# rg2/DeepFluoroLabeling-IPCAI2020

Measured on AMD Instinct MI355X. Metric: train images/sec, paper U-Net (depth 6, wf 5, BN, strided-conv down, seg + 14-landmark heads), 1x192x192 (8x-downsampled 184x184 padded), higher is better.
Workload: dtype bf16 (bf16 activations, activation gradients and GEMM weight copies in HBM; bf16 MFMA, fp32 accumulate, BatchNorm statistics, losses, weight gradients and master weights); 1 GPU; BASELINE configs[1]: 8x-downsampled, seg + 14-landmark heat-map dual head, batch 16 per GPU, Dice+NCC loss, SGD nesterov; global_batch=16, image=1x192x192, parallelism=dp1, math=bf16s, optimizer=dfl_amd.SGD(momentum 0.9, nesterov, wd 1e-4)

## Files before the change

### deepfluorolabeling-ipcai2020_amd/csrc/bn_elem.hip

```cpp
#include "chan_unit.h"

namespace dfl {

struct RowGeom {
  int UX;
  int gy;
};

static RowGeom row_geom(int C, int W) {
  const int units = C / W;
  RowGeom g;
  g.UX = 1;
  while (g.UX * 2 <= units && g.UX * 2 <= 256) g.UX *= 2;
  g.gy = (int)ceil_div(units, g.UX);
  return g;
}

static int rowblocks(int64_t M, int C) {
  int64_t nb = ceil_div(M * (int64_t)C, 8192);
  if (nb > 2048) nb = 2048;
  if (nb > M) nb = M;
  if (nb < 1) nb = 1;
  return (int)nb;
}

struct RowLane {
  int ux, uy, RY, c;
  bool cok;
  int64_t r0, r1;
};

template <int W>
__device__ __forceinline__ RowLane row_lane(int UX, int rows_per_block, int64_t M, int C) {
  RowLane t;
  t.RY = 256 / UX;
  t.ux = threadIdx.x % UX;
  t.uy = threadIdx.x / UX;
  t.c = (blockIdx.y * UX + t.ux) * W;
  t.cok = t.c < C;
  t.r0 = (int64_t)blockIdx.x * rows_per_block;
  t.r1 = t.r0 + rows_per_block;
  if (t.r1 > M) t.r1 = M;
  return t;
}

template <int NS, int W>
__device__ __forceinline__ void block_colsum(const float (&s)[NS][W], const RowLane& t, int UX, float* out, int C) {
  __shared__ float red[NS][256][W];
#pragma unroll
  for (int n = 0; n < NS; ++n)
#pragma unroll
    for (int j = 0; j < W; ++j) red[n][threadIdx.x][j] = s[n][j];
  __syncthreads();
  if (t.uy == 0 && t.cok) {
#pragma unroll
    for (int n = 0; n < NS; ++n)
#pragma unroll
      for (int j = 0; j < W; ++j) {
        float sum = 0.f;
        for (int y = 0; y < t.RY; ++y) sum += red[n][y * UX + t.ux][j];
        out[(int64_t)n * C + j] = sum;
      }
  }
}

template <int W, bool BF>
__global__ void __launch_bounds__(256) colstats_kernel(const dfl_colstats_args a, int UX, int rows_per_block) {
  using U = ChanUnit<W, BF>;
  const RowLane t = row_lane<W>(UX, rows_per_block, a.M, a.C);
  float s[2][W];
#pragma unroll
  for (int j = 0; j < W; ++j) s[0][j] = s[1][j] = 0.f;
  if (t.cok) {
    for (int64_t r = t.r0 + t.uy; r < t.r1; r += t.RY) {
      float va[W], vb[W];
      U::load(a.a, r * a.lda + t.c, va);
      if (a.b != nullptr) U::load(a.b, r * a.ldb + t.c, vb);
#pragma unroll
      for (int j = 0; j < W; ++j) {
        s[0][j] += va[j];
        s[1][j] = fmaf(va[j], a.b != nullptr ? vb[j] : va[j], s[1][j]);
      }
    }
  }
  block_colsum<2, W>(s, t, UX, a.partials + (int64_t)blockIdx.x * 2 * a.C + t.c, a.C);
}

__device__ __forceinline__ void sum_partials_f64(const float* __restrict__ partials, int nblocks, int C, int cpb,
                                                 double* out1, double* out2, double (*red)[256]) {
  const int cl = threadIdx.x % cpb, rl = threadIdx.x / cpb, lanes = 256 / cpb;
  const int c = blockIdx.x * cpb + cl;
  double s1 = 0.0, s2 = 0.0;
  if (c < C) {
    int r = rl;
    for (; r + 3 * lanes < nblocks; r += 4 * lanes) {
      float v1[4], v2[4];
#pragma unroll
      for (int u = 0; u < 4; ++u) {
        v1[u] = partials[((int64_t)(r + u * lanes) * 2 + 0) * C + c];
        v2[u] = partials[((int64_t)(r + u * lanes) * 2 + 1) * C + c];
      }
      s1 += ((double)v1[0] + (double)v1[1]) + ((double)v1[2] + (double)v1[3]);
      s2 += ((double)v2[0] + (double)v2[1]) + ((double)v2[2] + (double)v2[3]);
    }
    for (; r < nblocks; r += lanes) {
      s1 += (double)partials[((int64_t)r * 2 + 0) * C + c];
      s2 += (double)partials[((int64_t)r * 2 + 1) * C + c];
    }
  }
  for (int off = 32; off >= cpb; off >>= 1) {
    s1 += __shfl_xor(s1, off, 64);
    s2 += __shfl_xor(s2, off, 64);
  }
  const int wave = threadIdx.x >> 6, lane = threadIdx.x & 63;
  if (lane < cpb) {
    red[0][wave * 8 + lane] = s1;
    red[1][wave * 8 + lane] = s2;
  }
  __syncthreads();
  *out1 = (red[0][cl] + red[0][8 + cl]) + (red[0][16 + cl] + red[0][24 + cl]);
  *out2 = (red[1][cl] + red[1][8 + cl]) + (red[1][16 + cl] + red[1][24 + cl]);
}

static inline int finalize_cpb(int C) { return C >= 512 ? 8 : (C >= 256 ? 4 : (C >= 128 ? 2 : 1)); }

__global__ void __launch_bounds__(256) bn_finalize_kernel(const dfl_bn_finalize_args a, int cpb) {
  __shared__ double red[2][256];
  const int c = blockIdx.x * cpb + (threadIdx.x % cpb);
  double s1, s2;
  sum_partials_f64(a.partials, a.nblocks, a.C, cpb, &s1, &s2, red);
  if (threadIdx.x < cpb && c < a.C) {
    const double cnt = (double)a.count;
    const double mean = s1 / cnt;
    double var = s2 / cnt - mean * mean;
    if (var < 0.0) var = 0.0;
    const double invstd = 1.0 / sqrt(var + (double)a.eps);
    const float scale = (float)((double)a.gamma[c] * invstd);
    a.scale[c] = scale;
    a.shift[c] = (float)((double)a.beta[c] - mean * (double)a.gamma[c] * invstd);
    a.save_mean[c] = (float)mean;
    a.save_invstd[c] = (float)invstd;
    if (a.running_mean != nullptr) {
      const double mom = (double)a.momentum;
      const double unbiased = (cnt > 1.0) ? var * cnt / (cnt - 1.0) : var;
      a.running_mean[c] = (float)((1.0 - mom) * (double)a.running_mean[c] + mom * mean);
      a.running_var[c] = (float)((1.0 - mom) * (double)a.running_var[c] + mom * unbiased);
    }
  }
  if (blockIdx.x == 0 && threadIdx.x == 0 && a.num_batches_tracked != nullptr) *a.num_batches_tracked += 1;
}

__global__ void __launch_bounds__(256) bn_finalize_live_kernel(const dfl_bn_live_job* __restrict__ jobs) {
  const dfl_bn_live_job j = jobs[blockIdx.y];
  const int c = blockIdx.x * 256 + threadIdx.x;
  if (c < j.C) {
    float scale, shift;
    double mean, var;
    bn_live_affine(j.totals, j.gamma, j.beta, (double)j.count, j.eps, j.C, c, &scale, &shift, &mean, &var);
    j.scale[c] = scale;
    j.shift[c] = shift;
    j.save_mean[c] = (float)mean;
    j.save_invstd[c] = (float)(1.0 / sqrt(var + (double)j.eps));
    if (j.running_mean != nullptr) {
      const double mom = (double)j.momentum, cnt = (double)j.count;
      const double unbiased = (cnt > 1.0) ? var * cnt / (cnt - 1.0) : var;
      j.running_mean[c] = (float)((1.0 - mom) * (double)j.running_mean[c] + mom * mean);
      j.running_var[c] = (float)((1.0 - mom) * (double)j.running_var[c] + mom * unbiased);
    }
  }
  if (blockIdx.x == 0 && threadIdx.x == 0 && j.num_batches_tracked != nullptr) *j.num_batches_tracked += 1;
}

__global__ void __launch_bounds__(256) bn_bwd_finalize_live_kernel(const dfl_bn_bwd_live_job* __restrict__ jobs) {
  const dfl_bn_bwd_live_job j = jobs[blockIdx.y];
  const int c = blockIdx.x * 256 + threadIdx.x;
  if (c >= j.C) return;
  double sdy = 0.0, sdyr = 0.0;
#pragma unroll
  for (int r = 0; r < DFL_BN_R; ++r) {
    sdy += j.totals[(int64_t)(r * 2 + 0) * j.C + c];
    sdyr += j.totals[(int64_t)(r * 2 + 1) * j.C + c];
  }
  const double mean = (double)j.save_mean[c], invstd = (double)j.save_invstd[c];
  j.dgamma[c] = (float)(invstd * (sdyr - mean * sdy));
  j.dbeta[c] = (float)sdy;
  if (j.sum_out != nullptr) j.sum_out[c] = (float)sdy;
}

__global__ void bn_eval_kernel(const float* __restrict__ gamma, const float* __restrict__ beta,
                               const float* __restrict__ rm, const float* __restrict__ rv, float* __restrict__ scale,
                               float* __restrict__ shift, int C, float eps) {
  const int c = blockIdx.x * blockDim.x + threadIdx.x;
  if (c < C) {
    const float invstd = 1.0f / sqrtf(rv[c] + eps);
    const float s = gamma[c] * invstd;
    scale[c] = s;
    shift[c] = beta[c] - rm[c] * s;
  }
}

__global__ void __launch_bounds__(256) bn_bwd_finalize_kernel(const dfl_bn_bwd_finalize_args a, int cpb) {
  __shared__ double red[2][256];
  const int c = blockIdx.x * cpb + (threadIdx.x % cpb);
  double sdy, sdyr;
  sum_partials_f64(a.partials, a.nblocks, a.C, cpb, &sdy, &sdyr, red);
  if (threadIdx.x < cpb && c < a.C) {
    const double cnt = (double)a.count;
    const double mean = (double)a.save_mean[c], invstd = (double)a.save_invstd[c], g = (double)a.gamma[c];
    const double sdyx = invstd * (sdyr - mean * sdy);
    a.dgamma[c] = (float)sdyx;
    a.dbeta[c] = (float)sdy;
    const double s = g * invstd;
    const double c1 = a.count > 0 ? sdy / cnt : 0.0, c2 = a.count > 0 ? sdyx / cnt : 0.0;
    a.coef[0 * a.C + c] = (float)s;
    a.coef[1 * a.C + c] = (float)(-s * c2 * invstd);
    a.coef[2 * a.C + c] = (float)(-s * c1 + s * c2 * invstd * mean);
  }
}

template <int W, bool BF>
__global__ void __launch_bounds__(256) bn_relu_bwd_kernel(const dfl_bn_relu_bwd_args a, int UX, int rows_per_block) {
  using U = ChanUnit<W, BF>;
  const RowLane t = row_lane<W>(UX, rows_per_block, a.M, a.C);
  const int C = a.C, c = t.c, RY = t.RY;
  float cA[W], cB[W], cC[W], s[1][W];
#pragma unroll
  for (int j = 0; j < W; ++j) {
    cA[j] = 1.f; cB[j] = 0.f; cC[j] = 0.f; s[0][j] = 0.f;
    if (a.coef != nullptr && t.cok) {
      cA[j] = a.coef[c + j];
      cB[j] = a.coef[C + c + j];
      cC[j] = a.coef[2 * C + c + j];
    }
  }
  if (t.cok) {
    auto one = [&](const float* dy, const float* rv, int64_t r) {
      float o[W];
#pragma unroll
      for (int j = 0; j < W; ++j) o[j] = rv[j] > 0.f ? fmaf(cA[j], dy[j], fmaf(cB[j], rv[j], cC[j])) : 0.f;
      if (W == 4 && a.split_out) {
        if constexpr (W == 4) {
          uint2 parts[2];
          split_bf16<2>(make_float4(o[0], o[1], o[2], o[3]), parts);
          *reinterpret_cast<uint4*>(a.dpre + r * a.ldo + c) = make_uint4(parts[0].x, parts[0].y, parts[1].x, parts[1].y);
        }
      } else {
        U::store(a.dpre, r * a.ldo + c, o, o);
      }
#pragma unroll
      for (int j = 0; j < W; ++j) s[0][j] += o[j];
    };
    constexpr int R = (W == 4) ? 2 : 4;
    int64_t r = t.r0 + t.uy;
    for (; r + (R - 1) * RY < t.r1; r += R * RY) {
      float dy[R][W], rv[R][W];
#pragma unroll
      for (int u = 0; u < R; ++u) U::load(a.dy, (r + u * RY) * a.lddy + c, dy[u]);
#pragma unroll
      for (int u = 0; u < R; ++u) U::load(a.r, (r + u * RY) * a.ldr + c, rv[u]);
#pragma unroll
      for (int u = 0; u < R; ++u) one(dy[u], rv[u], r + u * RY);
    }
    for (; r < t.r1; r += RY) {
      float dy[W], rv[W];
      U::load(a.dy, r * a.lddy + c, dy);
      U::load(a.r, r * a.ldr + c, rv);
      one(dy, rv, r);
    }
  }
  if (a.partials == nullptr) return;
  block_colsum<1, W>(s, t, UX, a.partials + (int64_t)blockIdx.x * C + c, C);
}

__global__ void __launch_bounds__(256) reduce_partials_kernel(const float* __restrict__ partials, float* __restrict__ out,
                                                             int nblocks, int stride, int C) {
  __shared__ double red[256];
  const int cl = threadIdx.x & 7, rl = threadIdx.x >> 3;
  const int c = blockIdx.x * 8 + cl;
  double s = 0.0;
  if (c < C)
    for (int r = rl; r < nblocks; r += 32) s += (double)partials[(int64_t)r * stride + c];
  red[threadIdx.x] = s;
  __syncthreads();
  for (int off = 16; off >= 1; off >>= 1) {
    if (rl < off) red[threadIdx.x] += red[threadIdx.x + off * 8];
    __syncthreads();
  }
  if (threadIdx.x < 8 && c < C) out[c] = (float)red[threadIdx.x];
}

#ifndef DFL_RB_O
#define DFL_RB_O 32
#endif
constexpr int RB_T = 256, RB_O = DFL_RB_O, RB_S = 4 * RB_T / RB_O, RB_WIDE_MIN = 32;
static inline int reduce_job_blocks(int64_t n, int count) {
  return (int)(count >= RB_WIDE_MIN ? ceil_div(n, RB_O) : ceil_div(n, 4 * RB_T));
}

__device__ __forceinline__ void rb_load4(const float* __restrict__ p, int64_t i, int64_t n, bool vec, double* a) {
  if (vec) {
    const float4 v = *reinterpret_cast<const float4*>(p + i);
    a[0] += (double)v.x; a[1] += (double)v.y; a[2] += (double)v.z; a[3] += (double)v.w;
  } else {
#pragma unroll
    for (int e = 0; e < 4; ++e)
      if (i + e < n) a[e] += (double)p[i + e];
  }
}

__device__ __forceinline__ void rb_store4(const dfl_reduce_job& j, int64_t i, const double* v) {
#pragma unroll
  for (int e = 0; e < 4; ++e)
    if (i + e < j.n) {
      const int64_t ii = i + e;
      j.dst[j.T > 1 ? (ii % (j.n / j.T)) * j.T + ii / (j.n / j.T) : ii] = (float)v[e];
    }
}

__global__ void __launch_bounds__(RB_T) reduce_batch_kernel(const dfl_reduce_job* __restrict__ jobs, int njobs) {
  __shared__ double red[RB_S][RB_O + 2];
  int lo = 0, hi = njobs - 1;
  while (lo < hi) {
    const int mid = (lo + hi + 1) >> 1;
    if (jobs[mid].first_block <= (int)blockIdx.x) lo = mid; else hi = mid - 1;
  }
  const dfl_reduce_job j = jobs[lo];
  const int b = (int)blockIdx.x - j.first_block;
  const bool vec = (j.n & 3) == 0 && (j.stride & 3) == 0 && (reinterpret_cast<uintptr_t>(j.src) & 15) == 0;
  if (j.count >= RB_WIDE_MIN) {
    const int o4 = threadIdx.x % (RB_O / 4), sl = threadIdx.x / (RB_O / 4);
    const int64_t i = (int64_t)b * RB_O + 4 * o4;
    double a0[4] = {0, 0, 0, 0}, a1[4] = {0, 0, 0, 0}, a2[4] = {0, 0, 0, 0}, a3[4] = {0, 0, 0, 0};
    if (i < j.n) {
      int k = sl;
      if (vec) {
        for (; k + 7 * RB_S < j.count; k += 8 * RB_S) {
          float4 v[8];
#pragma unroll
          for (int u = 0; u < 8; ++u) v[u] = *reinterpret_cast<const float4*>(j.src + (int64_t)(k + u * RB_S) * j.stride + i);
#pragma unroll
          for (int u = 0; u < 8; u += 4) {
            a0[0] += (double)v[u].x; a0[1] += (double)v[u].y; a0[2] += (double)v[u].z; a0[3] += (double)v[u].w;
            a1[0] += (double)v[u + 1].x; a1[1] += (double)v[u + 1].y; a1[2] += (double)v[u + 1].z; a1[3] += (double)v[u + 1].w;
            a2[0] += (double)v[u + 2].x; a2[1] += (double)v[u + 2].y; a2[2] += (double)v[u + 2].z; a2[3] += (double)v[u + 2].w;
            a3[0] += (double)v[u + 3].x; a3[1] += (double)v[u + 3].y; a3[2] += (double)v[u + 3].z; a3[3] += (double)v[u + 3].w;
          }
        }
      }
      for (; k + 3 * RB_S < j.count; k += 4 * RB_S) {
        rb_load4(j.src + (int64_t)k * j.stride, i, j.n, vec, a0);
        rb_load4(j.src + (int64_t)(k + RB_S) * j.stride, i, j.n, vec, a1);
        rb_load4(j.src + (int64_t)(k + 2 * RB_S) * j.stride, i, j.n, vec, a2);
        rb_load4(j.src + (int64_t)(k + 3 * RB_S) * j.stride, i, j.n, vec, a3);
      }
      for (; k < j.count; k += RB_S) rb_load4(j.src + (int64_t)k * j.stride, i, j.n, vec, a0);
    }
#pragma unroll
    for (int e = 0; e < 4; ++e) red[sl][4 * o4 + e] = (a0[e] + a1[e]) + (a2[e] + a3[e]);
    __syncthreads();
    for (int off = RB_S / 2; off >= 1; off >>= 1) {
      if (sl < off) {
#pragma unroll
        for (int e = 0; e < 4; ++e) red[sl][4 * o4 + e] += red[sl + off][4 * o4 + e];
      }
      __syncthreads();
    }
    if (sl == 0 && i < j.n) rb_store4(j, i, &red[0][4 * o4]);
  } else {
    const int64_t i = ((int64_t)b * RB_T + threadIdx.x) * 4;
    if (i < j.n) {
      double s[4] = {0, 0, 0, 0};
      for (int k = 0; k < j.count; ++k) rb_load4(j.src + (int64_t)k * j.stride, i, j.n, vec, s);
      rb_store4(j, i, s);
    }
  }
}

template <int W, bool BF>
__global__ void __launch_bounds__(256) affine_copy_kernel(const dfl_affine_copy_args a, int64_t total_units, int cq) {
  using U = ChanUnit<W, BF>;
  const int64_t stride = (int64_t)gridDim.x * blockDim.x;
  for (int64_t i = (int64_t)blockIdx.x * blockDim.x + threadIdx.x; i < total_units; i += stride) {
    int u, xw, yh, n;
    unit_coords(i, cq, a.W, a.H, &u, &xw, &yh, &n);
    const int c = u * W;
    const int64_t so = (((int64_t)n * a.xH + a.xoy + yh) * a.xW + a.xox + xw) * a.ldx + c;
    const int64_t dof = (((int64_t)n * a.yH + a.yoy + yh) * a.yW + a.yox + xw) * a.ldy + c;
    float v[W];
    U::load(a.x, so, v);
    if (a.scale != nullptr) {
      float sc[W], sh[W];
      if constexpr (W == 4) {
        ChanUnit<4, false>::load(a.scale, c, sc);
        ChanUnit<4, false>::load(a.shift, c, sh);
      } else {
#pragma unroll
        for (int j = 0; j < W; ++j) { sc[j] = a.scale[c + j]; sh[j] = a.shift[c + j]; }
      }
#pragma unroll
      for (int j = 0; j < W; ++j) v[j] = fmaf(v[j], sc[j], sh[j]);
    }
    if (a.accumulate) {
      float o[W];
      U::load(a.y, dof, o);
#pragma unroll
      for (int j = 0; j < W; ++j) v[j] += o[j];
    }
    U::store(a.y, dof, v);
  }
}

__device__ __forceinline__ int64_t pool_src(const dfl_pool_args& a, int n, int oy, int ox, int ld) {
  return (((int64_t)n * a.H + 2 * oy) * a.W + 2 * ox) * ld;
}

template <int W, bool BF>
__global__ void __launch_bounds__(256) maxpool_fwd_kernel(const dfl_pool_args a, int64_t total_units, int cq) {
  using U = ChanUnit<W, BF>;
  const int Ho = a.H / 2, Wo = a.W / 2;
  const int64_t stride = (int64_t)gridDim.x * blockDim.x;
  for (int64_t i = (int64_t)blockIdx.x * blockDim.x + threadIdx.x; i < total_units; i += stride) {
    int u, ox, oy, n;
    unit_coords(i, cq, Wo, Ho, &u, &ox, &oy, &n);
    const int c = u * W;
    const int64_t s00 = pool_src(a, n, oy, ox, a.ldx) + c, s10 = s00 + (int64_t)a.W * a.ldx;
    float v0[W], v1[W], v2[W], v3[W], m[W];
    U::load(a.x, s00, v0);
    U::load(a.x, s00 + a.ldx, v1);
    U::load(a.x, s10, v2);
    U::load(a.x, s10 + a.ldx, v3);
#pragma unroll
    for (int j = 0; j < W; ++j) m[j] = fmaxf(fmaxf(v0[j], v1[j]), fmaxf(v2[j], v3[j]));
    U::store(a.y, (((int64_t)n * Ho + oy) * Wo + ox) * a.ldy + c, m);
  }
}

__device__ __forceinline__ int first_max4(float v0, float v1, float v2, float v3) {
  int k = 0;
  float m = v0;
  if (v1 > m) { m = v1; k = 1; }
  if (v2 > m) { m = v2; k = 2; }
  if (v3 > m) { k = 3; }
  return k;
}

template <int W, bool BF>
__global__ void __launch_bounds__(256) maxpool_bwd_kernel(const dfl_pool_args a, int64_t total_units, int cq) {
  using U = ChanUnit<W, BF>;
  const int Ho = a.H / 2, Wo = a.W / 2;
  const int64_t stride = (int64_t)gridDim.x * blockDim.x;
  for (int64_t i = (int64_t)blockIdx.x * blockDim.x + threadIdx.x; i < total_units; i += stride) {
    int u, ox, oy, n;
    unit_coords(i, cq, Wo, Ho, &u, &ox, &oy, &n);
    const int c = u * W;
    const int64_t s00 = pool_src(a, n, oy, ox, a.ldx) + c, s10 = s00 + (int64_t)a.W * a.ldx;
    const int64_t d00 = pool_src(a, n, oy, ox, a.lddx) + c, d10 = d00 + (int64_t)a.W * a.lddx;
    float v0[W], v1[W], v2[W], v3[W], g[W];
    U::load(a.x, s00, v0);
    U::load(a.x, s00 + a.ldx, v1);
    U::load(a.x, s10, v2);
    U::load(a.x, s10 + a.ldx, v3);
    U::load(a.y, (((int64_t)n * Ho + oy) * Wo + ox) * a.ldy + c, g);
    if constexpr (BF) {
      float e0[W], e1[W], e2[W], e3[W];
      U::load(a.dx, d00, e0);
      U::load(a.dx, d00 + a.lddx, e1);
      U::load(a.dx, d10, e2);
      U::load(a.dx, d10 + a.lddx, e3);
#pragma unroll
      for (int j = 0; j < W; ++j) {
        const int k = first_max4(v0[j], v1[j], v2[j], v3[j]);
        e0[j] += k == 0 ? g[j] : 0.f;
        e1[j] += k == 1 ? g[j] : 0.f;
        e2[j] += k == 2 ? g[j] : 0.f;
        e3[j] += k == 3 ? g[j] : 0.f;
      }
      U::store(a.dx, d00, e0);
      U::store(a.dx, d00 + a.lddx, e1);
      U::store(a.dx, d10, e2);
      U::store(a.dx, d10 + a.lddx, e3);
    } else {
#pragma unroll
      for (int j = 0; j < W; ++j) {
        const int k = first_max4(v0[j], v1[j], v2[j], v3[j]);
        a.dx[(k < 2 ? d00 : d10) + ((k & 1) ? a.lddx : 0) + j] += g[j];
      }
    }
  }
}

constexpr int PK_T = 32, PK_CMAX = 9;

__device__ __forceinline__ float pack_src(const dfl_pack_job& j, int k, int n) {
  int a, b, c;
  if (j.kind == 1) {
    c = k / j.B; b = k - c * j.B; a = n;
  } else if (j.kind == 2) {
    const int cp = k / j.A;
    a = k - cp * j.A; b = n; c = j.flip ? (j.C - 1 - cp) : cp;
  } else {
    a = k; c = n / j.B; b = n - c * j.B;
  }
  return j.src[((int64_t)a * j.B + b) * j.C + c];
}

__device__ __forceinline__ void pack_put(float* dst, int64_t q, int r, float v, int split) {
  if (!split) {
    dst[q * 4 + r] = v;
  } else {
    const __bf16 h = (__bf16)v;
    const __bf16 l = (__bf16)(v - (float)h);
    unsigned short* d16 = reinterpret_cast<unsigned short*>(dst) + q * 8;
    d16[r] = __builtin_bit_cast(unsigned short, h);
    d16[4 + r] = __builtin_bit_cast(unsigned short, l);
  }
}

__global__ void __launch_bounds__(256) pack_kernel(const dfl_pack_job* __restrict__ jobs) {
  __shared__ float tile[PK_T][PK_T * PK_CMAX + 1];
  const dfl_pack_job j = jobs[blockIdx.y];
  const int A = j.A, B = j.B, Cc = j.C;
  const int K = (j.kind == 1) ? Cc * B : (j.kind == 2 ? Cc * A : A);
  const int N = (j.kind == 1) ? A : (j.kind == 2 ? B : Cc * B);
  if (j.split == 2 && Cc <= PK_CMAX && ((j.kind == 1) ? (B % 16 == 0) : (A % 16 == 0))) {
    const int tb = (B + PK_T - 1) / PK_T, ta = (A + PK_T - 1) / PK_T;
    const int run = PK_T * Cc;
    unsigned short* dst16 = reinterpret_cast<unsigned short*>(j.dst);
    for (int tidx = blockIdx.x; tidx < ta * tb; tidx += gridDim.x) {
      const int a0 = (tidx / tb) * PK_T, b0 = (tidx % tb) * PK_T;
      const int nb = min(PK_T, B - b0), na = min(PK_T, A - a0);
      __syncthreads();
      for (int e = threadIdx.x; e < PK_T * run; e += 256) {
        const int ar = e / run, q = e - ar * run;
        if (ar < na && q < nb * Cc) tile[ar][q] = j.src[((int64_t)(a0 + ar) * B + b0) * Cc + q];
      }
      __syncthreads();
      for (int e = threadIdx.x; e < 64 * Cc; e += 256) {
        const int x = e & 31, blk = (e >> 5) & 1, cp = e >> 6;
        float f[16];
        int64_t cell;
        bool ok;
        if (j.kind == 1) {
          ok = x < na && 16 * blk < nb;
#pragma unroll
          for (int r = 0; r < 16; ++r) f[r] = tile[x][(16 * blk + r) * Cc + cp];
          cell = (int64_t)((cp * B + b0) / 16 + blk) * N + a0 + x;
        } else if (j.kind == 2) {
          const int c = j.flip ? (Cc - 1 - cp) : cp;
          ok = x < nb && 16 * blk < na;
#pragma unroll
          for (int r = 0; r < 16; ++r) f[r] = tile[16 * blk + r][x * Cc + c];
          cell = (int64_t)((cp * A + a0) / 16 + blk) * N + b0 + x;
        } else {
          ok = x < nb && 16 * blk < na;
#pragma unroll
          for (int r = 0; r < 16; ++r) f[r] = tile[16 * blk + r][x * Cc + cp];
          cell = (int64_t)(a0 / 16 + blk) * N + cp * B + b0 + x;
        }
        if (ok) {
          u32x4* d = reinterpret_cast<u32x4*>(dst16 + cell * 16);
          d[0] = pack8(f);
          d[1] = pack8(f + 8);
        }
      }
    }
    return;
  }
  if (j.split == 2) {
    const int Kc = (K + 15) / 16;
    const int64_t cells = (int64_t)Kc * N;
    const int64_t stride = (int64_t)gridDim.x * blockDim.x;
    for (int64_t i = (int64_t)blockIdx.x * blockDim.x + threadIdx.x; i < cells; i += stride) {
      const int n = (int)(i % N), kc = (int)(i / N);
      float f[16];
#pragma unroll
      for (int r = 0; r < 16; ++r) {
        const int k = kc * 16 + r;
        f[r] = k < K ? pack_src(j, k, n) : 0.f;
      }
      u32x4* d = reinterpret_cast<u32x4*>(reinterpret_cast<unsigned short*>(j.dst) + i * 16);
      d[0] = pack8(f);
      d[1] = pack8(f + 8);
    }
    return;
  }
  const bool tiled = Cc <= PK_CMAX && ((j.kind == 1) ? (B % 4 == 0) : (A % 4 == 0));
  if (tiled) {
    const int tb = (B + PK_T - 1) / PK_T, ta = (A + PK_T - 1) / PK_T;
    const int run = PK_T * Cc;
    for (int tidx = blockIdx.x; tidx < ta * tb; tidx += gridDim.x) {
      const int a0 = (tidx / tb) * PK_T, b0 = (tidx % tb) * PK_T;
      const int nb = min(PK_T, B - b0), na = min(PK_T, A - a0);
      __syncthreads();
      for (int e = threadIdx.x; e < PK_T * run; e += 256) {
        const int ar = e / run, q = e - ar * run;
        if (ar < na && q < nb * Cc) tile[ar][q] = j.src[((int64_t)(a0 + ar) * B + b0) * Cc + q];
      }
      __syncthreads();
      for (int e = threadIdx.x; e < PK_T * run; e += 256) {
        const int r = e & 3, x = (e >> 2) & 31, rest = e >> 7;
        if (j.kind == 1) {
          const int c = rest >> 3, bq = rest & 7, bb = 4 * bq + r, ar = x;
          if (ar < na && bb < nb)
            pack_put(j.dst, (int64_t)((c * B + b0) / 4 + bq) * N + a0 + ar, r, tile[ar][bb * Cc + c], j.split);
        } else if (j.kind == 2) {
          const int cp = rest >> 3, aq = rest & 7, ar = 4 * aq + r, bb = x;
          const int c = j.flip ? (Cc - 1 - cp) : cp;
          if (ar < na && bb < nb)
            pack_put(j.dst, (int64_t)((cp * A + a0) / 4 + aq) * N + b0 + bb, r, tile[ar][bb * Cc + c], j.split);
        } else {
          const int c = rest >> 3, aq = rest & 7, ar = 4 * aq + r, bb = x;
          if (ar < na && bb < nb)
            pack_put(j.dst, (int64_t)(a0 / 4 + aq) * N + c * B + b0 + bb, r, tile[ar][bb * Cc + c], j.split);
        }
      }
    }
    return;
  }
  const int Kq = (K + 3) / 4;
  const int64_t total = (int64_t)Kq * N * 4;
  const int64_t stride = (int64_t)gridDim.x * blockDim.x;
  for (int64_t i = (int64_t)blockIdx.x * blockDim.x + threadIdx.x; i < total; i += stride) {
    const int r = (int)(i & 3);
    const int64_t t = i >> 2;
    const int n = (int)(t % N), kq = (int)(t / N);
    const int k = 4 * kq + r;
    pack_put(j.dst, i >> 2, r, (k < K) ? pack_src(j, k, n) : 0.f, j.split);
  }
}

__device__ __forceinline__ void pack_emit_cells(const float (*tile)[PK_T * PK_CMAX + 1], unsigned short* dst16, int kind, int flip,
                                                int A, int B, int Cc, int a0, int b0) {
  const int N = (kind == 1) ? A : (kind == 2 ? B : Cc * B);
  for (int e = threadIdx.x; e < 64 * Cc; e += 256) {
    const int x = e & 31, blk = (e >> 5) & 1, cp = e >> 6;
    float f[16];
    int64_t cell;
    if (kind == 1) {
#pragma unroll
      for (int r = 0; r < 16; ++r) f[r] = tile[x][(16 * blk + r) * Cc + cp];
      cell = (int64_t)((cp * B + b0) / 16 + blk) * N + a0 + x;
    } else if (kind == 2) {
      const int c = flip ? (Cc - 1 - cp) : cp;
#pragma unroll
      for (int r = 0; r < 16; ++r) f[r] = tile[16 * blk + r][x * Cc + c];
      cell = (int64_t)((cp * A + a0) / 16 + blk) * N + b0 + x;
    } else {
#pragma unroll
      for (int r = 0; r < 16; ++r) f[r] = tile[16 * blk + r][x * Cc + cp];
      cell = (int64_t)(a0 / 16 + blk) * N + cp * B + b0 + x;
    }
    u32x4* d = reinterpret_cast<u32x4*>(dst16 + cell * 16);
    d[0] = pack8(f);
    d[1] = pack8(f + 8);
  }
}

__device__ __forceinline__ void pack_emit_quads(const float (*tile)[PK_T * PK_CMAX + 1], float* dst, int kind, int flip, int split,
                                                int A, int B, int Cc, int a0, int b0) {
  const int N = (kind == 1) ? A : (kind == 2 ? B : Cc * B);
  const int run = PK_T * Cc;
  for (int e = threadIdx.x; e < PK_T * run; e += 256) {
    const int r = e & 3, x = (e >> 2) & 31, rest = e >> 7;
    if (kind == 1) {
      const int c = rest >> 3, bq = rest & 7, bb = 4 * bq + r, ar = x;
      pack_put(dst, (int64_t)((c * B + b0) / 4 + bq) * N + a0 + ar, r, tile[ar][bb * Cc + c], split);
    } else if (kind == 2) {
      const int cp = rest >> 3, aq = rest & 7, ar = 4 * aq + r, bb = x;
      const int c = flip ? (Cc - 1 - cp) : cp;
      pack_put(dst, (int64_t)((cp * A + a0) / 4 + aq) * N + b0 + bb, r, tile[ar][bb * Cc + c], split);
    } else {
      const int c = rest >> 3, aq = rest & 7, ar = 4 * aq + r, bb = x;
      pack_put(dst, (int64_t)(a0 / 4 + aq) * N + c * B + b0 + bb, r, tile[ar][bb * Cc + c], split);
    }
  }
// ... 391 lines not shown
```

Before: 4681 images/sec.

## Restructure batched partial-sum reduction with wave shuffles and transposed-output staging

Rewrites reduce_batch_kernel, which sums weight-gradient partials. Job lookup becomes a wave ballot instead of a binary search. The wide path now uses a configurable number of slice lanes per wave with shuffle reductions before a smaller LDS tree, and predicated unrolled rounds of loads. A new narrow path for transposed outputs stages results in shared memory so the stores are coalesced, and the plain narrow path unrolls its loads. The aim is to reduce LDS traffic, barrier count, scattered transposed writes and load latency, at the cost of more complex code with inline asm and scheduling barriers.

```diff
diff --git a/deepfluorolabeling-ipcai2020_amd/csrc/bn_elem.hip b/deepfluorolabeling-ipcai2020_amd/csrc/bn_elem.hip
--- a/deepfluorolabeling-ipcai2020_amd/csrc/bn_elem.hip
+++ b/deepfluorolabeling-ipcai2020_amd/csrc/bn_elem.hip
@@ -289,18 +289,32 @@
   if (threadIdx.x < 8 && c < C) out[c] = (float)red[threadIdx.x];
 }
 
-#ifndef DFL_RB_O
-#define DFL_RB_O 32
+#ifndef DFL_RB_P
+#define DFL_RB_P 8
 #endif
-constexpr int RB_T = 256, RB_O = DFL_RB_O, RB_S = 4 * RB_T / RB_O, RB_WIDE_MIN = 32;
+#ifndef DFL_RB_G
+#define DFL_RB_G 1
+#endif
+constexpr int RB_S = 32, RB_P = DFL_RB_P, RB_L = 64 / RB_P, RB_W = RB_S / RB_P, RB_GO = 4 * RB_L, RB_G = DFL_RB_G;
+constexpr int RB_O = RB_GO * RB_G, RB_T = 64 * RB_W * RB_G, RB_WIDE_MIN = 32;
+static_assert((RB_P == 2 || RB_P == 4 || RB_P == 8) && RB_T <= 1024, "2, 4 or 8 slice lanes per wave");
 static inline int reduce_job_blocks(int64_t n, int count) {
   return (int)(count >= RB_WIDE_MIN ? ceil_div(n, RB_O) : ceil_div(n, 4 * RB_T));
 }
 
+__device__ __forceinline__ void rb_add4(double* a, const float4& v) {
+  a[0] += (double)v.x; a[1] += (double)v.y; a[2] += (double)v.z; a[3] += (double)v.w;
+}
+
+__device__ __forceinline__ float4 rb_ld16(const float* p) {
+  typedef float f4 __attribute__((ext_vector_type(4)));
+  const f4 v = *(const f4 __attribute__((address_space(1))) *)(uintptr_t)p;
+  return make_float4(v.x, v.y, v.z, v.w);
+}
+
 __device__ __forceinline__ void rb_load4(const float* __restrict__ p, int64_t i, int64_t n, bool vec, double* a) {
   if (vec) {
-    const float4 v = *reinterpret_cast<const float4*>(p + i);
-    a[0] += (double)v.x; a[1] += (double)v.y; a[2] += (double)v.z; a[3] += (double)v.w;
+    rb_add4(a, rb_ld16(p + i));
   } else {
 #pragma unroll
     for (int e = 0; e < 4; ++e)
@@ -308,69 +322,171 @@
   }
 }
 
+template <int R>
+__device__ __forceinline__ void rb_round(const float* p, const float* q, int64_t stride, int left, double* a0, double* a1,
+                                         double* a2, double* a3) {
+  if (R == 8) asm volatile("; round of eight"); else asm volatile("; round of four");
+  float4 v[R];
+#pragma unroll
+  for (int u = 0; u < R; ++u) v[u] = rb_ld16(u < left ? q + (int64_t)(u * RB_S) * stride : p);
+  __builtin_amdgcn_sched_barrier(0);
+#pragma unroll
+  for (int u = 0; u < R; ++u)
+    asm volatile("" : "+v"(v[u].x), "+v"(v[u].y), "+v"(v[u].z), "+v"(v[u].w));
+#pragma unroll
+  for (int u = 0; u < R; ++u) {
+    v[u].x = u < left ? v[u].x : 0.f; v[u].y = u < left ? v[u].y : 0.f;
+    v[u].z = u < left ? v[u].z : 0.f; v[u].w = u < left ? v[u].w : 0.f;
+  }
+  if (R == 8 && left >= 8) {
+#pragma unroll
+    for (int u = 0; u < R; u += 4) { rb_add4(a0, v[u]); rb_add4(a1, v[u + 1]); rb_add4(a2, v[u + 2]); rb_add4(a3, v[u + 3]); }
+  } else if (left >= 4) {
+    rb_add4(a0, v[0]); rb_add4(a1, v[1]); rb_add4(a2, v[2]); rb_add4(a3, v[3]);
+#pragma unroll
+    for (int u = 4; u < 7 && u < R; ++u) rb_add4(a0, v[u]);
+  } else {
+#pragma unroll
+    for (int u = 0; u < 3; ++u) rb_add4(a0, v[u]);
+  }
+}
+
+__device__ __forceinline__ void rb_walk(const float* p, int64_t stride, int count, double* s) {
+  int k = 0;
+  for (; k + 3 < count; k += 4) {
+    float4 v[4];
+#pragma unroll
+    for (int u = 0; u < 4; ++u) v[u] = rb_ld16(p + (int64_t)(k + u) * stride);
+#pragma unroll
+    for (int u = 0; u < 4; ++u) rb_add4(s, v[u]);
+  }
+  if (k < count) {
+    float4 v[3];
+#pragma unroll
+    for (int u = 0; u < 3; ++u) {
+      v[u] = rb_ld16(p + (int64_t)(k + u < count ? k + u : k) * stride);
+      if (k + u >= count) v[u] = make_float4(0.f, 0.f, 0.f, 0.f);
+    }
+#pragma unroll
+    for (int u = 0; u < 3; ++u) rb_add4(s, v[u]);
+  }
+}
+
 __device__ __forceinline__ void rb_store4(const dfl_reduce_job& j, int64_t i, const double* v) {
-#pragma unroll
-  for (int e = 0; e < 4; ++e)
-    if (i + e < j.n) {
-      const int64_t ii = i + e;
-      j.dst[j.T > 1 ? (ii % (j.n / j.T)) * j.T + ii / (j.n / j.T) : ii] = (float)v[e];
-    }
-}
-
-__global__ void __launch_bounds__(RB_T) reduce_batch_kernel(const dfl_reduce_job* __restrict__ jobs, int njobs) {
-  __shared__ double red[RB_S][RB_O + 2];
-  int lo = 0, hi = njobs - 1;
-  while (lo < hi) {
-    const int mid = (lo + hi + 1) >> 1;
-    if (jobs[mid].first_block <= (int)blockIdx.x) lo = mid; else hi = mid - 1;
-  }
-  const dfl_reduce_job j = jobs[lo];
+  if (j.T > 1) {
+    const int64_t m = j.n / j.T;
+    int64_t t = i / m, r = i - t * m;
+#pragma unroll
+    for (int e = 0; e < 4; ++e)
+      if (i + e < j.n) {
+        j.dst[r * j.T + t] = (float)v[e];
+        if (++r == m) { r = 0; ++t; }
+      }
+  } else if (i + 3 < j.n && (reinterpret_cast<uintptr_t>(j.dst + i) & 15) == 0) {
+    *reinterpret_cast<float4*>(j.dst + i) = make_float4((float)v[0], (float)v[1], (float)v[2], (float)v[3]);
+  } else {
+#pragma unroll
+    for (int e = 0; e < 4; ++e)
+      if (i + e < j.n) j.dst[i + e] = (float)v[e];
+  }
+}
+
+__global__ void __launch_bounds__(RB_T) __attribute__((amdgpu_waves_per_eu(4, 8))) reduce_batch_kernel(const dfl_reduce_job* __restrict__ jobs, int njobs) {
+  __shared__ double red[RB_G][RB_W][RB_GO];
+  const int lane = threadIdx.x & 63, wv = threadIdx.x >> 6;
+  int below = 0;
+  for (int base = 0; base < njobs; base += 64) {
+    const bool le = base + lane < njobs && jobs[base + lane].first_block <= (int)blockIdx.x;
+    below += __popcll(__ballot(le));
+  }
+  const dfl_reduce_job j = jobs[__builtin_amdgcn_readfirstlane(below - 1)];
   const int b = (int)blockIdx.x - j.first_block;
   const bool vec = (j.n & 3) == 0 && (j.stride & 3) == 0 && (reinterpret_cast<uintptr_t>(j.src) & 15) == 0;
   if (j.count >= RB_WIDE_MIN) {
-    const int o4 = threadIdx.x % (RB_O / 4), sl = threadIdx.x / (RB_O / 4);
-    const int64_t i = (int64_t)b * RB_O + 4 * o4;
+    const int o4 = lane % RB_L, w = __builtin_amdgcn_readfirstlane(wv) % RB_W, og = wv / RB_W, sl = w + RB_W * (lane / RB_L);
+    const int64_t i = (int64_t)b * RB_O + RB_GO * og + 4 * o4;
     double a0[4] = {0, 0, 0, 0}, a1[4] = {0, 0, 0, 0}, a2[4] = {0, 0, 0, 0}, a3[4] = {0, 0, 0, 0};
     if (i < j.n) {
       int k = sl;
       if (vec) {
-        for (; k + 7 * RB_S < j.count; k += 8 * RB_S) {
-          float4 v[8];
-#pragma unroll
-          for (int u = 0; u < 8; ++u) v[u] = *reinterpret_cast<const float4*>(j.src + (int64_t)(k + u * RB_S) * j.stride + i);
-#pragma unroll
-          for (int u = 0; u < 8; u += 4) {
-            a0[0] += (double)v[u].x; a0[1] += (double)v[u].y; a0[2] += (double)v[u].z; a0[3] += (double)v[u].w;
-            a1[0] += (double)v[u + 1].x; a1[1] += (double)v[u + 1].y; a1[2] += (double)v[u + 1].z; a1[3] += (double)v[u + 1].w;
-            a2[0] += (double)v[u + 2].x; a2[1] += (double)v[u + 2].y; a2[2] += (double)v[u + 2].z; a2[3] += (double)v[u + 2].w;
-            a3[0] += (double)v[u + 3].x; a3[1] += (double)v[u + 3].y; a3[2] += (double)v[u + 3].z; a3[3] += (double)v[u + 3].w;
-          }
+        const float* p = j.src + i + (int64_t)sl * j.stride;
+        const int mine = (j.count - 1 - sl) / RB_S + 1, most = (j.count - 1 - w) / RB_S + 1;
+        for (int done = 0; done < most; done += 8) {
+          const float* q = p + (int64_t)(done * RB_S) * j.stride;
+          const int left = mine - done;
+          if (most - done > 4) rb_round<8>(p, q, j.stride, left, a0, a1, a2, a3);
+          else rb_round<4>(p, q, j.stride, left, a0, a1, a2, a3);
         }
-      }
-      for (; k + 3 * RB_S < j.count; k += 4 * RB_S) {
-        rb_load4(j.src + (int64_t)k * j.stride, i, j.n, vec, a0);
-        rb_load4(j.src + (int64_t)(k + RB_S) * j.stride, i, j.n, vec, a1);
-        rb_load4(j.src + (int64_t)(k + 2 * RB_S) * j.stride, i, j.n, vec, a2);
-        rb_load4(j.src + (int64_t)(k + 3 * RB_S) * j.stride, i, j.n, vec, a3);
-      }
-      for (; k < j.count; k += RB_S) rb_load4(j.src + (int64_t)k * j.stride, i, j.n, vec, a0);
-    }
-#pragma unroll
-    for (int e = 0; e < 4; ++e) red[sl][4 * o4 + e] = (a0[e] + a1[e]) + (a2[e] + a3[e]);
+      } else {
+        for (; k + 3 * RB_S < j.count; k += 4 * RB_S) {
+          rb_load4(j.src + (int64_t)k * j.stride, i, j.n, false, a0);
+          rb_load4(j.src + (int64_t)(k + RB_S) * j.stride, i, j.n, false, a1);
+          rb_load4(j.src + (int64_t)(k + 2 * RB_S) * j.stride, i, j.n, false, a2);
+          rb_load4(j.src + (int64_t)(k + 3 * RB_S) * j.stride, i, j.n, false, a3);
+        }
+        for (; k < j.count; k += RB_S) rb_load4(j.src + (int64_t)k * j.stride, i, j.n, false, a0);
+      }
+    }
+#pragma unroll
+    for (int e = 0; e < 4; ++e) {
+      double s = (a0[e] + a1[e]) + (a2[e] + a3[e]);
+#pragma unroll
+      for (int off = RB_P / 2; off >= 1; off >>= 1) s += __shfl_down(s, off * RB_L);
+      if (lane < RB_L) red[og][w][4 * o4 + e] = s;
+    }
     __syncthreads();
-    for (int off = RB_S / 2; off >= 1; off >>= 1) {
-      if (sl < off) {
-#pragma unroll
-        for (int e = 0; e < 4; ++e) red[sl][4 * o4 + e] += red[sl + off][4 * o4 + e];
+    const int64_t ii = (int64_t)b * RB_O + threadIdx.x;
+    if (threadIdx.x < RB_O && ii < j.n) {
+      double r[RB_W];
+#pragma unroll
+      for (int u = 0; u < RB_W; ++u) r[u] = red[threadIdx.x / RB_GO][u][threadIdx.x % RB_GO];
+#pragma unroll
+      for (int off = RB_W / 2; off >= 1; off >>= 1) {
+#pragma unroll
+        for (int u = 0; u < off; ++u) r[u] += r[u + off];
+      }
+      int64_t o = ii;
+      if (j.T > 1) {
+        if (j.n <= 0x7fffffff) {
+          const unsigned m = (unsigned)j.n / (unsigned)j.T, t = (unsigned)ii / m;
+          o = (int64_t)((unsigned)ii - t * m) * j.T + t;
+        } else {
+          const int64_t m = j.n / j.T;
+          o = (ii % m) * j.T + ii / m;
+        }
+      }
+      j.dst[o] = (float)r[0];
+    }
+  } else if (vec && j.T > 1 && j.T <= 64 && ((j.n / j.T) & 3) == 0) {
+    __shared__ __attribute__((aligned(16))) float stage[4 * RB_T];
+    const int T = j.T, R = (4 * RB_T / T) & ~3;
+    const int64_t m = j.n / T, nchunks = (m + R - 1) / R, nblocks = (j.n + 4 * RB_T - 1) / (4 * RB_T);
+    for (int64_t c = b; c < nchunks; c += nblocks) {
+      const int64_t r0 = c * R;
+      const int rows = (int)(m - r0 < R ? m - r0 : R), rq = rows >> 2;
+      if ((int)threadIdx.x < T * rq) {
+        const int t = threadIdx.x / rq, r4 = threadIdx.x - t * rq;
+        double s[4] = {0, 0, 0, 0};
+        rb_walk(j.src + t * m + r0 + 4 * r4, j.stride, j.count, s);
+#pragma unroll
+        for (int e = 0; e < 4; ++e) stage[(4 * r4 + e) * T + t] = (float)s[e];
       }
       __syncthreads();
-    }
-    if (sl == 0 && i < j.n) rb_store4(j, i, &red[0][4 * o4]);
+      float* out = j.dst + r0 * T;
+      if ((reinterpret_cast<uintptr_t>(out) & 15) == 0) {
+        for (int y = threadIdx.x; y < rows * T / 4; y += RB_T) reinterpret_cast<float4*>(out)[y] = reinterpret_cast<const float4*>(stage)[y];
+      } else {
+        for (int y = threadIdx.x; y < rows * T; y += RB_T) out[y] = stage[y];
+      }
+      __syncthreads();
+    }
   } else {
     const int64_t i = ((int64_t)b * RB_T + threadIdx.x) * 4;
     if (i < j.n) {
       double s[4] = {0, 0, 0, 0};
-      for (int k = 0; k < j.count; ++k) rb_load4(j.src + (int64_t)k * j.stride, i, j.n, vec, s);
+      if (vec) rb_walk(j.src + i, j.stride, j.count, s);
+      else
+        for (int k = 0; k < j.count; ++k) rb_load4(j.src + (int64_t)k * j.stride, i, j.n, false, s);
       rb_store4(j, i, s);
     }
   }
```

Measured after the change: 4715 images/sec, median of 6. No clear change (+0.7%).
